# albireo77/moonrtx

Hardware: AMD Instinct MI355X
Metric: Mrays/s (primary camera samples) at 3840x2160, 64 spp, downscale-2 DEM (higher is better)
Workload: dtype f32

## Files before the change

moonrtx_amd/csrc/mrtx_kernels.hip:

```cpp
#include <hip/hip_runtime.h>
#include <stdint.h>
#include <string.h>
#include <stdlib.h>
#include <type_traits>

#include "mrtx_device.h"
#include "mrtx_march.h"

namespace mrtx {

#ifdef MRTX_PROF
__device__ unsigned long long g_prof[16];
#endif

__device__ __forceinline__ uint32_t mix32(uint32_t x) {
    x ^= x >> 16; x *= 0x7feb352dU;
    x ^= x >> 15; x *= 0x846ca68bU;
    x ^= x >> 16;
    return x;
}
__device__ __forceinline__ float u01(uint32_t key, uint32_t dim) {
    const uint32_t r = mix32(key + (dim + 1u) * 0x9E3779B9u);
    return (float)(r >> 8) * 5.9604644775390625e-08f;
}
// ... 165 lines not shown
        if (!have) {
            const bool far_end = !(y <= 0.0f);
            const float q0 = far_end ? o0 - ba0 : o0, q1 = far_end ? o1 - ba1 : o1, q2 = far_end ? o2 - ba2 : o2;
            const float B2 = fmaf(dz, q2, fmaf(dy, q1, dx * q0));
            const float C2 = fmaf(q2, q2, fmaf(q1, q1, q0 * q0)) - rr;
            const float h2 = fmaf(B2, B2, -C2);
            if (h2 > 0.0f) { cand = -B2 - sqrtf(h2); have = true; }
        }
        if (have) {
            const float sc = ta + cand;
            if (sc > smin && sc < best) { best = sc; which = k; }
        }
    }
    return which >= 0 ? best : -1.0e30f;
}


__device__ __forceinline__ void env_rowcol(const FrameC& f, float fx, float fy, float& rowf, float& colf) {
    const float sx = fmaf(fx, CF(f)->two_over_w, -1.0f);
    const float sy = fmaf(-fy, CF(f)->two_over_h, 1.0f);
    float dx = fmaf(sy, CF(f)->Vy[0], fmaf(sx, CF(f)->Ux[0], CF(f)->Wd[0]));
    float dy = fmaf(sy, CF(f)->Vy[1], fmaf(sx, CF(f)->Ux[1], CF(f)->Wd[1]));
    float dz = fmaf(sy, CF(f)->Vy[2], fmaf(sx, CF(f)->Ux[2], CF(f)->Wd[2]));
    const float inv_len = rcp_cr(sqrt_sh(fmaf(dz, dz, fmaf(dy, dy, dx * dx))));
    dx = dx * inv_len; dy = dy * inv_len; dz = dz * inv_len;
    float el, az;
    latlon(dx, dy, dz, fmaf(dy, dy, dx * dx), el, az);
    rowf = fmaf(el, CF(f)->bg_row_scale, CF(f)->bg_row_off);
    colf = fmaf(az, CF(f)->bg_col_scale, CF(f)->bg_col_off);
}
__device__ __forceinline__ bool sky_pixel_uniform(const FrameC& f, int x, int y, float& e0, float& e1, float& e2) {
    float r00, c00, r10, c10, r01, c01, r11, c11;
    const float fx = (float)x, fy = (float)y;
    env_rowcol(f, fx, fy, r00, c00);
    env_rowcol(f, fx + 1.0f, fy, r10, c10);
    env_rowcol(f, fx, fy + 1.0f, r01, c01);
    env_rowcol(f, fx + 1.0f, fy + 1.0f, r11, c11);
    const float m = fmaf(1.0e-6f, (float)max(CF(f)->bg_w, CF(f)->bg_h), 0.02f);
    const float rlo = fminf(fminf(r00, r10), fminf(r01, r11)) - m, rhi = fmaxf(fmaxf(r00, r10), fmaxf(r01, r11)) + m;
    const float clo = fminf(fminf(c00, c10), fminf(c01, c11)) - m, chi = fmaxf(fmaxf(c00, c10), fmaxf(c01, c11)) + m;
    const float rf = floorf(rlo), cf = floorf(clo);
    const bool uni = rf == floorf(rhi) && cf == floorf(chi) && rlo >= 0.0f && clo >= 0.0f &&
                     rhi < (float)CF(f)->bg_h && chi < (float)CF(f)->bg_w;
    e0 = e1 = e2 = 0.0f;
    if (uni) {
        const uint32_t px = reinterpret_cast<const uint32_t*>(CF(f)->bg)[(int64_t)(int)rf * CF(f)->bg_w + (int)cf];
        e0 = (float)(px & 255u) * kInv255;
        e1 = (float)((px >> 8) & 255u) * kInv255;
        e2 = (float)((px >> 16) & 255u) * kInv255;
    }
    return uni;
}

#define MRTX_PARK_SLOTS 4
__device__ __forceinline__ void park_put(v4f* park, int slot, float a, float b, float c, float d) {
    const v4f v = {a, b, c, d};
    park[slot * 64 + threadIdx.x] = v;
}
__device__ __forceinline__ v4f park_get(const v4f* park, int slot) { return park[slot * 64 + threadIdx.x]; }
__device__ __forceinline__ void park_fence() { asm volatile("" ::: "memory"); }

struct SampleOut {
    float c0, c1, c2, hitflag;
    float h0, h1, h2, h3;
    float oa, ob, oc, da, db, dc, t0, t1, t2, row, col;
    uint32_t ks, aux;
    bool path;
};

template <bool STATS, bool WIDE, int MODE, bool OVERLAY>
__device__ __forceinline__ void trace_sample(const FrameC& f, int lt, int x, int y, uint32_t gs, SampleOut& o,
                                             uint32_t* cnt, bool lead = false, v4f* park = nullptr) {
    constexpr bool BOUNCE = MODE == 1, DEFER = MODE == 2;
    auto emit_hit = [&](float h0, float h1, float h2, float h3) {
        if (DEFER) {
            if (lead) reinterpret_cast<float4*>(CF(f)->hits)[(int64_t)y * f.W + x] = make_float4(h0, h1, h2, h3);
        } else {
            o.h0 = h0; o.h1 = h1; o.h2 = h2; o.h3 = h3;
        }
    };
    constexpr int BATCH = BOUNCE ? MRTX_STEP_BATCH_BOUNCE : MRTX_STEP_BATCH;
    const uint32_t pix = (uint32_t)y * (uint32_t)f.W + (uint32_t)x;
    const uint32_t kp = mix32(pix + CF(f)->key0);
    const uint32_t ks = mix32(kp ^ (gs * 0x85EBCA6Bu + 1u));
    const float u0 = u01(ks, 0), u1 = u01(ks, 1), u2 = u01(ks, 2), u3 = u01(ks, 3);
    o.c0 = o.c1 = o.c2 = 0.0f; o.hitflag = 0.0f;
    o.h0 = o.h1 = o.h2 = o.h3 = 0.0f;
    o.path = false;
    if (DEFER) { o.oa = o.ob = o.oc = o.da = o.db = o.dc = o.t0 = o.t1 = o.t2 = o.row = o.col = 0.0f; o.ks = 0u; o.aux = 0u; }
    if (STATS) cnt[ST_PRIMARY]++;
    PROF_BEGIN(1);

    const float fx = (float)x + u0, fy = (float)y + u1;
    const float sx = fmaf(fx, CF(f)->two_over_w, -1.0f);
    const float sy = fmaf(-fy, CF(f)->two_over_h, 1.0f);
    float dx = fmaf(sy, CF(f)->Vy[0], fmaf(sx, CF(f)->Ux[0], CF(f)->Wd[0]));
    float dy = fmaf(sy, CF(f)->Vy[1], fmaf(sx, CF(f)->Ux[1], CF(f)->Wd[1]));
    float dz = fmaf(sy, CF(f)->Vy[2], fmaf(sx, CF(f)->Ux[2], CF(f)->Wd[2]));
    const float inv_len = rcp_cr(sqrt_sh(fmaf(dz, dz, fmaf(dy, dy, dx * dx))));
    dx = dx * inv_len; dy = dy * inv_len; dz = dz * inv_len;
    if (MODE == 3) {
        if (CF(f)->bg) env_lookup<STATS>(f, dx, dy, dz, o.c0, o.c1, o.c2, cnt);
        emit_hit(0.0f, 0.0f, 0.0f, 0.0f);
        return;
    }

    const double Dx = (double)dx, Dy = (double)dy, Dz = (double)dz;
    const double a = (Dx * Dx + Dy * Dy) + Dz * Dz;
    const double b = (CF(f)->oc[0] * Dx + CF(f)->oc[1] * Dy) + CF(f)->oc[2] * Dz;
    const double disc = b * b - a * CF(f)->cq;
    bool on_sphere = false;
    double t0 = 0.0, t1 = 0.0;
    if (disc > 0.0) {
        const double sq = (double)sqrtf((float)disc);
        const double inva = (double)rcp_cr((float)a);
        t0 = (-b - sq) * inva;
        t1 = (-b + sq) * inva;
        if (t1 > 0.0) { on_sphere = true; if (t0 < 0.0) t0 = 0.0; }
    }
    int cap = -1;
    float cap_s = 0.0f, cr0 = 0.0f, cr1 = 0.0f, cr2 = 0.0f;
    double tc0 = 0.0;
    bool cap_front = false;
    if (OVERLAY) {
        tc0 = -b * (double)rcp_cr((float)a);
// ... 64 lines not shown
             CF(f)->centerf[1] + fmaf(v.pc, CF(f)->Mf[2][1], fmaf(v.pb, CF(f)->Mf[1][1], v.pa * CF(f)->Mf[0][1])),
             CF(f)->centerf[2] + fmaf(v.pc, CF(f)->Mf[2][2], fmaf(v.pb, CF(f)->Mf[1][2], v.pa * CF(f)->Mf[0][2])),
             (float)t0 + lo);

    float t0r = 1.0f, t1r = 1.0f, t2r = 1.0f;
    uint32_t seg = 1;
    float ul1 = u2, ul2 = u3;
    uint32_t ksl = ks;
    float org_row = 0.0f, org_col = 0.0f, org_cell = 0.0f;
    for (;;) {
        PROF_BEGIN(5);
        float wgt;
        if (DEFER) {
            float oa, ob, oc, wa, wb, wc, carried = 0.0f;
            const bool have_s = light_sample(f, v, ul1, ul2, oa, ob, oc, wa, wb, wc, carried);
            float q2o;
            exact_rowcol(f, oa, ob, oc, org_row, org_col, q2o);
            org_cell = CF(f)->hmip != nullptr ? horizon_cell(f, org_row, org_col) : 0.0f;
            park_put(park, 3, org_row, org_col, org_cell, 0.0f);
            park_put(park, 0, v.pa, v.pb, v.pc, v.na);
            park_put(park, 1, v.nb, v.nc, v.al0, v.al1);
            park_put(park, 2, v.al2, __uint_as_float(ksl), carried, 0.0f);
            park_fence();
            bool occluded = false;
            if (have_s) {
                if (STATS) cnt[ST_SHADOW]++;
                Seg ssg;
                float sk_occ;
                MarchState ms;
                ms.rowA = org_row; ms.colA = org_col;
                bool sgo = march_begin_at<false, STATS, false, true>(f, oa, ob, oc, wa, wb, wc, ms, cnt, org_cell);
                while (sgo) march_segment<WIDE, false, STATS, MRTX_SHADOW_BATCH, 2>(f, ms, 0.0f, ssg, sgo, occluded, sk_occ, cnt);
            }
            park_fence();
            { const v4f p3 = park_get(park, 3); org_row = p3.x; org_col = p3.y; org_cell = p3.z; }
            const v4f p0 = park_get(park, 0), p1 = park_get(park, 1), p2 = park_get(park, 2);
            v.pa = p0.x; v.pb = p0.y; v.pc = p0.z; v.na = p0.w;
            v.nb = p1.x; v.nc = p1.y; v.al0 = p1.z; v.al1 = p1.w;
            v.al2 = p2.x; ksl = __float_as_uint(p2.y);
            wgt = (have_s && !occluded) ? p2.z : 0.0f;
        } else {
            wgt = direct_light<STATS, WIDE, BATCH>(f, v, ul1, ul2, cnt);
        }
        PROF_END(5);
        o.c0 = fmaf(t0r * v.al0, wgt, o.c0);
        o.c1 = fmaf(t1r * v.al1, wgt, o.c1);
        o.c2 = fmaf(t2r * v.al2, wgt, o.c2);
        if (DEFER) {
            if (continue_path(f, v, ksl, 1u, t0r, t1r, t2r, o.oa, o.ob, o.oc, o.da, o.db, o.dc)) {
                o.row = org_row; o.col = org_col;
                o.t0 = t0r; o.t1 = t1r; o.t2 = t2r;
                o.ks = ksl; o.aux = 0u;
                if (STATS) cnt[ST_BOUNCE]++;
#ifdef MRTX_PROF
                uint32_t tcnt[16];
#pragma unroll
                for (int i = 0; i < 16; i++) tcnt[i] = 0;
#else
                uint32_t tcnt_store[STATS ? ST_N : 1];
                uint32_t* const tcnt = STATS ? tcnt_store : nullptr;
#endif
                if (STATS) {
#pragma unroll
                    for (int i = 0; i < ST_N; i++) tcnt[i] = 0;
                }
                MarchState tm;
                tm.rowA = o.row; tm.colA = o.col;
                park_put(park, 0, o.c0, o.c1, o.c2, o.t0);
                park_put(park, 1, o.t1, o.t2, __uint_as_float(o.ks), 0.0f);
                park_fence();
                bool tgo = march_begin_at<false, STATS, false, true>(f, o.oa, o.ob, o.oc, o.da, o.db, o.dc, tm, tcnt, org_cell);
                bool thit = false;
                Seg tsg;
                float tsk = 0.0f;
                if (tgo) march_segment<WIDE, false, STATS, MRTX_TRIAL_BATCH, 3>(f, tm, 0.0f, tsg, tgo, thit, tsk, tcnt);
                park_fence();
                const v4f p0 = park_get(park, 0), p1 = park_get(park, 1);
                o.c0 = p0.x; o.c1 = p0.y; o.c2 = p0.z; o.t0 = p0.w;
                o.t1 = p1.x; o.t2 = p1.y; o.ks = __float_as_uint(p1.z);
                t0r = o.t0; t1r = o.t1; t2r = o.t2;
#ifdef MRTX_PROF_TRIAL
                cnt[13] += tcnt[11]; cnt[14] += tcnt[12]; cnt[15] += tcnt[6] + tcnt[7];
#endif
                if (STATS) {
#pragma unroll
                    for (int i = 0; i < ST_N; i++) cnt[i] += tcnt[i];
                }
                if (!tgo && !thit) {
                    escaped_path<STATS>(f, o.oa, o.ob, o.oc, o.da, o.db, o.dc, t0r, t1r, t2r, o.c0, o.c1, o.c2, cnt);
                } else {
                    o.path = true;
                    if (thit) {
                        o.aux = MRTX_REC_HIT | ((uint32_t)(int)rintf(tsk * f.inv_step) << 8);
                    } else {
                        o.aux = MRTX_REC_RESUME | ((uint32_t)tm.kend << 8);
                        o.row = tm.rowA; o.col = tm.colA;
                    }
                }
            }
        }
        if (!BOUNCE) break;
        float boa, bob, boc, bda, bdb, bdc;
        if (!continue_path(f, v, ks, seg, t0r, t1r, t2r, boa, bob, boc, bda, bdb, bdc)) break;
        const uint32_t d0 = 4u + 5u * (seg - 1u);
        ul1 = u01(ks, d0 + 3u); ul2 = u01(ks, d0 + 4u);
        if (STATS) cnt[ST_BOUNCE]++;
        Seg bsg;
        float bhi = 0.0f;
        if (!march<WIDE, false, STATS, BATCH>(f, boa, bob, boc, bda, bdb, bdc, 0.0f, bsg, bhi, cnt)) {
            escaped_path<STATS>(f, boa, bob, boc, bda, bdb, bdc, t0r, t1r, t2r, o.c0, o.c1, o.c2, cnt);
            break;
        }
        const int bk = (int)rintf(bhi * f.inv_step);
        float blo = (float)(bk - 1) * f.step;
        refine<WIDE>(f, bsg, boa, bob, boc, bda, bdb, bdc, blo, bhi);
        if (STATS) { cnt[ST_HEIGHT] += (uint32_t)f.nbis; cnt[ST_FETCH] += (uint32_t)f.nbis; }
        hit_vertex<STATS, WIDE>(f, fmaf(blo, bda, boa), fmaf(blo, bdb, bob), fmaf(blo, bdc, boc), v, cnt);
        seg++;
    }
}

template <int S>
__device__ __forceinline__ float tree_sum(float v) {
#pragma unroll
    for (int m = 1; m < S; m <<= 1) v += __shfl_xor(v, m, 64);
    return v;
}

#ifndef MRTX_WG_TILE
#define MRTX_WG_TILE 1
#endif
#ifndef MRTX_SKY_WG_TILE
#define MRTX_SKY_WG_TILE 8
#endif
#ifndef MRTX_MIN_WAVES
#define MRTX_MIN_WAVES 4
#endif
#ifndef MRTX_XCD_SHARE
#define MRTX_XCD_SHARE 1
#endif
#ifndef MRTX_XCD_TILE_RUN
#define MRTX_XCD_TILE_RUN 1
#endif
#ifndef MRTX_XCD_SHARE_BELOW
#define MRTX_XCD_SHARE_BELOW 1200
#endif
#ifndef MRTX_MIN_WAVES_BOUNCE
#define MRTX_MIN_WAVES_BOUNCE 5
#endif
#ifndef MRTX_BOUNCE_STATS_WAVES
#define MRTX_BOUNCE_STATS_WAVES 2
#endif
#define MRTX_BOUNCE_WAVES(STATS, SV) ((STATS) ? MRTX_BOUNCE_STATS_WAVES : ((SV) <= 2 ? 4 : MRTX_MIN_WAVES_BOUNCE))
template <int S, bool STATS, bool WIDE, int MODE, bool OVERLAY>
#ifndef MRTX_MIN_WAVES_DEFER
#define MRTX_MIN_WAVES_DEFER 3
#endif
__global__ void __launch_bounds__(64, MODE == 1 ? MRTX_BOUNCE_WAVES(STATS, S) : MODE == 2 ? MRTX_MIN_WAVES_DEFER : MRTX_MIN_WAVES)
render_kernel(const FrameC f, const PathQ pq) {
    constexpr bool DEFER = MODE == 2;
    constexpr int P = 64 / S;
    constexpr int PW = P >= 64 ? 8 : P >= 32 ? 8 : P >= 16 ? 4 : P >= 8 ? 4 : P >= 4 ? 2 : P >= 2 ? 2 : 1;
    constexpr int PH = P / PW;
    constexpr int WGTILE = MODE == 3 ? MRTX_SKY_WG_TILE : MRTX_WG_TILE;
    constexpr int WGT = (PW > WGTILE) ? PW : WGTILE;
    constexpr int WGS = WGT == 16 ? 4 : WGT == 8 ? 3 : WGT == 4 ? 2 : WGT == 2 ? 1 : 0;
    constexpr int JX = WGT / PW, JY = WGT / PH, NJOBS = JX * JY;
    __shared__ unsigned int lds_cnt[ST_N];
    __shared__ v4f park_lds[DEFER ? MRTX_PARK_SLOTS * 64 : 1];
    v4f* const park = DEFER ? park_lds : nullptr;

    const int lane = threadIdx.x & 63, wv = threadIdx.x >> 6;
    const int subs_x = f.tile_w >> WGS, subs = subs_x * (f.tile_h >> WGS);
    const int b = blockIdx.x, xcd = b & 7, g = b >> 3;
    int li, sub;
    if (f.xcd_share) {
        const int per = subs >> 3;
        li = g / per; sub = xcd * per + g % per;
    } else {
        constexpr int K = MRTX_XCD_TILE_RUN;
        const int rem = g % (subs * K);
        li = ((g / (subs * K)) * 8 + xcd) * K + rem / subs; sub = rem % subs;
    }
    if (li >= f.n_active) return;
    const int lt = f.tile_list ? f.tile_list[li] : li;
    const int t = lt * f.world + f.rank;
    int tx, ty;
    mrtx_tile_xy(t, f.tiles_x, f.tile_shift, tx, ty);
    const int px0 = tx * f.tile_w + (sub % subs_x) * WGT, py0 = ty * f.tile_h + (sub / subs_x) * WGT;
    if (px0 >= f.W || py0 >= f.H) return;

#ifdef MRTX_PROF
    uint32_t cnt[16];
    if (!STATS) {
#pragma unroll
        for (int i = 0; i < 16; i++) cnt[i] = 0;
    }
#else
    uint32_t cnt_store[STATS ? ST_N : 1];
    uint32_t* const cnt = STATS ? cnt_store : nullptr;
#endif
    if (STATS) {
#pragma unroll
        for (int i = 0; i < ST_N; i++) cnt[i] = 0;
        if (threadIdx.x < ST_N) lds_cnt[threadIdx.x] = 0;
        __syncthreads();
    }

    const int p = lane / S, s = lane % S;
    constexpr bool SKY_UNI = MODE == 3 && WGT == 8;
    uint64_t sky_nu = ~0ull;
    auto sky_jobmask = [&](int jx_, int jy_) {
        uint64_t mk = 0ull;
#pragma unroll
        for (int r = 0; r < PH; r++) mk |= (uint64_t)((1u << PW) - 1u) << ((jy_ * PH + r) * 8 + jx_ * PW);
        return mk;
    };
    if (SKY_UNI && CF(f)->bg != nullptr) {
        const int ux = px0 + (lane & 7), uy = py0 + (lane >> 3);
        const bool uin = ux < f.W && uy < f.H;
        float sky0, sky1, sky2;
        const bool uni = sky_pixel_uniform(f, ux, uy, sky0, sky1, sky2);
        sky_nu = __ballot(uin && !uni);
        if (uin && (sky_nu & sky_jobmask((lane & 7) / PW, (lane >> 3) / PH)) == 0ull) {
            const int64_t upix = (int64_t)uy * f.W + ux;
            float4 a = make_float4(0.f, 0.f, 0.f, 0.f);
            if (f.first_block != 0) a = reinterpret_cast<const float4*>(CF(f)->accum)[upix];
            const float b0 = (float)S * sky0, b1 = (float)S * sky1, b2 = (float)S * sky2;
            a.x += b0; a.y += b1; a.z += b2; a.w += 0.0f;
            reinterpret_cast<float4*>(CF(f)->accum)[upix] = a;
            reinterpret_cast<float4*>(CF(f)->hits)[upix] = make_float4(0.f, 0.f, 0.f, 0.f);
            if (STATS) { cnt[ST_PRIMARY] += (uint32_t)S; cnt[ST_BG] += (uint32_t)S; }
        }
    }
    for (int job = wv; job < NJOBS; job++) {
        const int jx = job % JX, jy = job / JX;
        const int x = px0 + jx * PW + (p % PW), y = py0 + jy * PH + (p / PW);
        if (px0 + jx * PW >= f.W || py0 + jy * PH >= f.H) continue;
        if (SKY_UNI && (sky_nu & sky_jobmask(jx, jy)) == 0ull) continue;
        const bool inb = x < f.W && y < f.H;
        float s0 = 0.f, s1 = 0.f, s2 = 0.f, s3 = 0.f;
        SampleOut o;
        o.h0 = o.h1 = o.h2 = o.h3 = 0.f;
        o.path = false;
        o.oa = o.ob = o.oc = o.da = o.db = o.dc = o.t0 = o.t1 = o.t2 = o.row = o.col = 0.f; o.ks = 0u; o.aux = 0u;
        bool deferred = false;
        constexpr uint32_t n_blk = 1u;
        for (uint32_t blk = 0; blk < n_blk; blk++) {
            o.c0 = o.c1 = o.c2 = o.hitflag = 0.f;
            PROF_BEGIN(0);
            if (inb) trace_sample<STATS, WIDE, MODE, OVERLAY>(f, lt, x, y, (f.first_block + blk) * (uint32_t)S + (uint32_t)s, o, cnt, s == 0, park);
            PROF_END(0);
            if (blk == 0 && f.first_block != 0 && inb && s == 0) {
                const float4 prev = reinterpret_cast<const float4*>(CF(f)->accum)[(int64_t)y * f.W + x];
                s0 = prev.x; s1 = prev.y; s2 = prev.z; s3 = prev.w;
            }
            if (DEFER) deferred = __ballot(o.path) != 0ull;
            if (DEFER && deferred) {
                const uint32_t chunk = (uint32_t)blockIdx.x * (uint32_t)NJOBS + (uint32_t)job;
                const uint32_t e = chunk * 64u + (uint32_t)lane;
                const uint64_t pm = __ballot(o.path);
                const uint32_t es = chunk * 64u + __builtin_amdgcn_mbcnt_hi((uint32_t)(pm >> 32), __builtin_amdgcn_mbcnt_lo((uint32_t)pm, 0u));
                if (o.path) {
                    nt_store4(pq.ray0 + es, o.oa, o.ob, o.oc, o.da);
                    nt_store4(pq.ray1 + es, o.db, o.dc, o.t0, o.t1);
                    nt_store4(pq.ray2 + es, o.t2, o.row, o.col, __uint_as_float(o.ks));
                    pq.lane_of[es] = (uint32_t)lane | o.aux;
                }
                { float* const cp = reinterpret_cast<float*>(pq.c4) + 3u * (size_t)e;
                  __builtin_nontemporal_store(o.c0, cp); __builtin_nontemporal_store(o.c1, cp + 1); __builtin_nontemporal_store(o.c2, cp + 2); }
                if (lane == 0) pq.npaths[chunk] = (uint8_t)__popcll(pm);
                if (lane == 0) pq.meta[chunk] = 0x80000000u | (uint32_t)(px0 + jx * PW) | ((uint32_t)(py0 + jy * PH) << 15);
            } else {
                s0 += tree_sum<S>(o.c0);
                s1 += tree_sum<S>(o.c1);
                s2 += tree_sum<S>(o.c2);
            }
            s3 += tree_sum<S>(o.hitflag);
        }
        if (inb && s == 0) reinterpret_cast<float4*>(CF(f)->accum)[(int64_t)y * f.W + x] = make_float4(s0, s1, s2, s3);
        if (!DEFER && inb && s == 0) reinterpret_cast<float4*>(CF(f)->hits)[(int64_t)y * f.W + x] = make_float4(o.h0, o.h1, o.h2, o.h3);
    }

#ifdef MRTX_PROF
    if (!STATS && lane == 0 && (((uint32_t)(blockIdx.x >> 3) * 2654435761u) >> 26) == 0u) {
        cnt[10] = 1;
#pragma unroll
        for (int i = 0; i < 16; i++) atomicAdd(&g_prof[i], (unsigned long long)cnt[i]);
    }
#endif
    if (STATS) {
#pragma unroll
        for (int i = 0; i < ST_N; i++) {
            uint32_t v = cnt[i];
#pragma unroll
            for (int m = 1; m < 64; m <<= 1) v += __shfl_xor(v, m, 64);
            if (lane == 0) atomicAdd(&lds_cnt[i], v);
        }
        __syncthreads();
        if (threadIdx.x < ST_N) atomicAdd(&CF(f)->stats[threadIdx.x], (unsigned long long)lds_cnt[threadIdx.x]);
    }
}

#ifndef MRTX_PATH_WAVES
#define MRTX_PATH_WAVES 5
#endif
#ifndef MRTX_PATH_STEPS
#define MRTX_PATH_STEPS 2
#endif
#ifdef MRTX_PATH_PROF
__device__ unsigned long long g_pprof[16];
__device__ unsigned long long g_pprof_end[8192];
__device__ unsigned long long g_pprof_t[16];
#endif
enum { PS_IDLE = 0, PS_NEEDSEG, PS_STEP, PS_BISECT, PS_ENDED, PS_HITWAIT, PS_SHADE, PS_ESCAPED };

template <bool STATS>
__device__ __forceinline__ uint32_t step_mask(const FrameC& f, const MarchState& m, const Seg& sg, uint32_t todo, uint32_t* cnt) {
    const float* m2 = CF(f)->mip2;
    const int pitch = CF(f)->m2_pitch, sh = CF(f)->m2_shift, mh = CF(f)->m2_h, mw = CF(f)->m2_w;
    uint32_t rem = todo, keep = 0u;
    while (rem != 0u) {
        int jj[4]; bool on[4]; float mv[4];
#pragma unroll
        for (int q = 0; q < 4; q++) {
            on[q] = rem != 0u;
            jj[q] = on[q] ? (int)__builtin_ctz(rem) + 1 : 1;
            rem &= rem - 1u;
        }
#pragma unroll
        for (int q = 0; q < 4; q++) {
            const float u = ((float)(m.ka + jj[q]) * f.step - sg.sa) * f.inv_step;
            const float rowf = fmaf(u, fmaf(u, sg.r2, sg.r1), sg.ra), colf = fmaf(u, fmaf(u, sg.c2, sg.c1), sg.ca);
            int i = ((int)floorf(rowf) >> sh) + 1, c = ((int)floorf(colf) >> sh) + 1;
            i = max(0, min(i, mh + 1)); c = max(0, min(c, mw + 1));
            mv[q] = on[q] ? m2[i * pitch + c] : 0.0f;
        }
        if (STATS) { cnt[ST_MIP] += (on[0] ? 1u : 0u) + (on[1] ? 1u : 0u) + (on[2] ? 1u : 0u) + (on[3] ? 1u : 0u); }
#pragma unroll
        for (int q = 0; q < 4; q++) {
            const float sk = (float)(m.ka + jj[q]) * f.step;
            const float pa = fmaf(sk, m.da, m.oa), pb = fmaf(sk, m.db, m.ob), pc = fmaf(sk, m.dc, m.oc);
            const float r2 = fmaf(pc, pc, fmaf(pb, pb, pa * pa));
            const float rd = f.Rf * mv[q];
            if (on[q] && r2 <= (rd * rd) * 1.00001f) keep |= 1u << (jj[q] - 1);
        }
    }
    return keep;
}

template <bool STATS, bool WIDE>
__global__ void __launch_bounds__(64, STATS ? 2 : MRTX_PATH_WAVES) path_kernel(const FrameC f, const PathQ pq) {
    const uint32_t lane = threadIdx.x;
    const uint32_t label = blockIdx.x & 7u;
    const uint32_t sub = (blockIdx.x >> 3) % (uint32_t)pq.n_sub;
// ... 725 lines not shown
        int i = t / mp - 1, j = t % mp - 1;
        i = i < 0 ? 0 : (i > mh - 1 ? mh - 1 : i);
        j = j < 0 ? mw - 1 : (j > mw - 1 ? 0 : j);
        const int r0 = max(C * i - 2, -2), r1 = min(C * i + C + 1, h + 1);
        const int c0 = max(C * j - 2, -2), c1 = min(C * j + C + 1, w + 1);
        float m = 0.0f;
        for (int r = r0; r <= r1; r++) {
            const float* row = dem_padded + ((int64_t)(r + 2) * pitch + 2) * (MRTX_DEM_ELEM_BYTES / 4);
            for (int c = c0; c <= c1; c++) m = fmaxf(m, row[c * (MRTX_DEM_ELEM_BYTES / 4)]);
        }
        mip[t] = m;
    }
}

__global__ void hmip_build_kernel(const float* __restrict__ mip, int mh, int mw, int shift, float* __restrict__ out,
                                  int hh, int hw, int hshift, int h, int w) {
    const int mp = mw + 2, Cc = 1 << hshift;
    for (int t = blockIdx.x * blockDim.x + threadIdx.x; t < hh * hw; t += gridDim.x * blockDim.x) {
        const int i = t / hw, j = t % hw;
        const int r0 = max(Cc * i - Cc, 0), r1 = min(Cc * i + 2 * Cc - 1, h - 1);
        const int c0 = Cc * j - Cc, c1 = Cc * j + 2 * Cc - 1;
        float m = 0.0f;
        int a0 = 0, a1 = mw - 1, b0 = 1, b1 = 0;
        if (c1 - c0 + 1 < w) {
            if (c0 < 0)       { a0 = (c0 + w) >> shift; a1 = mw - 1; b0 = 0; b1 = c1 >> shift; }
            else if (c1 >= w) { a0 = c0 >> shift; a1 = mw - 1; b0 = 0; b1 = (c1 - w) >> shift; }
            else              { a0 = c0 >> shift; a1 = c1 >> shift; }
        }
        for (int fi = r0 >> shift; fi <= (r1 >> shift); fi++) {
            for (int fj = a0; fj <= a1; fj++) m = fmaxf(m, mip[(fi + 1) * mp + fj + 1]);
            for (int fj = b0; fj <= b1; fj++) m = fmaxf(m, mip[(fi + 1) * mp + fj + 1]);
        }
        out[t] = m;
    }
}

__global__ void mip_pair_kernel(const float* __restrict__ mip, float2* __restrict__ out, int rows, int pitch) {
    const int n = rows * pitch;
    for (int t = blockIdx.x * blockDim.x + threadIdx.x; t < n; t += gridDim.x * blockDim.x) {
        const int r = t / pitch;
        out[t] = make_float2(mip[t], mip[r + 1 < rows ? t + pitch : t]);
    }
}

}

#ifdef MRTX_DEV_ONE
#ifndef MRTX_DEV_ONE_MODE
#define MRTX_DEV_ONE_MODE 2
#endif
#if MRTX_DEV_ONE_MODE == 9
template __global__ void mrtx::path_kernel<false, true>(const FrameC, const PathQ);
#else
template __global__ void mrtx::render_kernel<64, false, true, MRTX_DEV_ONE_MODE, false>(const FrameC, const PathQ);
#endif
#else
extern "C++" {
static void render_geometry(const FrameC& f, int S, int& xcd_share, unsigned& grid, int& njobs, int& pw_log2, int mode = 0) {
    const int P = 64 / S;
    const int PW = P >= 32 ? 8 : P >= 8 ? 4 : P >= 2 ? 2 : 1;
    const int PH = P / PW;
    const int wgtile = mode == 3 ? MRTX_SKY_WG_TILE : MRTX_WG_TILE;
    const int wgt = (PW > wgtile) ? PW : wgtile;
    const int subs = (f.tile_w / wgt) * (f.tile_h / wgt);
    xcd_share = (MRTX_XCD_SHARE && (subs & 7) == 0 && f.n_active < MRTX_XCD_SHARE_BELOW) ? 1 : 0;
    const int groups = xcd_share ? f.n_active : (f.n_active + 8 * MRTX_XCD_TILE_RUN - 1) / (8 * MRTX_XCD_TILE_RUN) * (8 * MRTX_XCD_TILE_RUN);
    grid = (unsigned)(groups * subs);
    njobs = (wgt / PW) * (wgt / PH);
    pw_log2 = PW == 8 ? 3 : PW == 4 ? 2 : PW == 2 ? 1 : 0;
}
uint64_t mrtx_path_chunks(const FrameC& f, int S, uint32_t* grid_a, int* njobs_log2) {
    int share, njobs, pwl; unsigned grid;
    render_geometry(f, S, share, grid, njobs, pwl);
    if (grid_a) *grid_a = grid;
    if (njobs_log2) *njobs_log2 = njobs == 2 ? 1 : 0;
    return (uint64_t)grid * (uint64_t)njobs;
}
hipError_t mrtx_launch_render(const FrameC& f, int S, bool stats, int mode, bool overlay, const PathQ* pq, hipStream_t st) {
    FrameC fr = f;
    int njobs, pwl; unsigned gx;
    render_geometry(f, S, fr.xcd_share, gx, njobs, pwl, mode);
    const dim3 grid(gx), block(64);
    if (f.n_blocks != 1) return hipErrorInvalidValue;
    if (grid.x == 0) return hipSuccess;
    PathQ q;
    memset(&q, 0, sizeof q);
    if (mode == 2) {
        if (!pq || pq->n_chunks != (uint64_t)gx * (uint64_t)njobs || pq->grid_a != gx || (1 << pq->njobs_log2) != njobs)
            return hipErrorInvalidValue;
        q = *pq;
    }
    const bool wide = f.dem_wide != 0;
    static const unsigned dev_lds = getenv("MOONRT_DEV_LDS") ? (unsigned)atoi(getenv("MOONRT_DEV_LDS")) : 0u;
#define MRTX_LAUNCH(SV, ST, WD, MD, OV) hipLaunchKernelGGL((mrtx::render_kernel<SV, ST, WD, MD, OV>), grid, block, dev_lds, st, fr, q)
#define MRTX_CASE3(SV, MD, OV)                                                                                     \
        if (wide) { if (stats) MRTX_LAUNCH(SV, true, true, MD, OV); else MRTX_LAUNCH(SV, false, true, MD, OV); }   \
        else { if (stats) MRTX_LAUNCH(SV, true, false, MD, OV); else MRTX_LAUNCH(SV, false, false, MD, OV); }
#define MRTX_CASE2(SV, MD) if (overlay) { MRTX_CASE3(SV, MD, true) } else { MRTX_CASE3(SV, MD, false) }
#define MRTX_CASE(SV)                                                  \
    case SV:                                                           \
        if (mode == 1) { MRTX_CASE2(SV, 1) } else if (mode == 2) { MRTX_CASE2(SV, 2) }                              \
        else if (mode == 3) { if (stats) MRTX_LAUNCH(SV, true, false, 3, false); else MRTX_LAUNCH(SV, false, false, 3, false); }   \
        else { MRTX_CASE2(SV, 0) }   \
        break;
    switch (S) {
#ifndef MRTX_DEV_ONLY_S64
        MRTX_CASE(1) MRTX_CASE(2) MRTX_CASE(4) MRTX_CASE(8) MRTX_CASE(16) MRTX_CASE(32)
// ... 206 lines not shown
```

moonrtx_amd/csrc/mrtx_march.h:

```cpp
#pragma once
#include <hip/hip_runtime.h>
#include <stdint.h>

#include "mrtx_device.h"

#define CF(f) ((const __attribute__((address_space(4))) FrameCold*)(f).cold)

#ifndef MRTX_TRIAL_BATCH
#define MRTX_TRIAL_BATCH 1
#endif

namespace mrtx {

__device__ constexpr float kPi = 3.14159274101257324f;
__device__ constexpr float kHalfPi = 1.57079637050628662f;
__device__ constexpr float kInv255 = 0.003921568859368563f;

#ifdef MRTX_PROF
#ifdef MRTX_PROF_FULLIV
#define PROF_BEGIN(i)
#define PROF_END(i)
#else
#define PROF_BEGIN(i) const unsigned long long _pt##i = __builtin_readcyclecounter()
#define PROF_END(i) cnt[i] += (uint32_t)(__builtin_readcyclecounter() - _pt##i)
// ... 469 lines not shown
            mv[q] = m2[min((uint32_t)((i + 1) * pitch + c + 1), maxidx)];
        }
        bool found = false;
#pragma unroll
        for (int q = 0; q < Q; q++) {
            const int jj = j - q;
            const float sk = fmaf((float)max(jj, sg.jlo), f.step, sg.sa);
            const float r2 = fmaf(sk, fmaf(sk, m.rq.a, two_b), m.rq.q0);
            const float rd = f.Rf * mv[q];
            const bool kept = !(r2 > (rd * rd) * 1.00001f);
            if (STATS) cnt[ST_MIP] += (!found && jj >= sg.jlo) ? 1u : 0u;
            if (!found && jj >= sg.jlo && kept) { last = jj; found = true; }
        }
        j -= Q;
        open = !found && j >= sg.jlo;
    }
    return last;
}
template <bool STATS, int Q>
__device__ __forceinline__ int first_kept_step(const FrameC& f, const MarchState& m, const Seg& sg, uint32_t* cnt) {
    const float* m2 = CF(f)->mip2;
    const int pitch = CF(f)->m2_pitch, sh = CF(f)->m2_shift;
    const uint32_t maxidx = (uint32_t)((CF(f)->m2_h + 2) * pitch - 1);
    const float two_b = m.rq.b + m.rq.b;
    int j = sg.jlo;
    int first = sg.jlo;
    bool open = (sg.jlo <= sg.jhi) & !sg.exact;
    if (open) first = sg.jhi + 1;
    while (open) {
        float mv[Q];
#pragma unroll
        for (int q = 0; q < Q; q++) {
            const float u = (float)min(j + q, sg.jhi);
            const float rowf = fmaf(u, fmaf(u, sg.r2, sg.r1), sg.ra), colf = fmaf(u, fmaf(u, sg.c2, sg.c1), sg.ca);
            const int i = (int)floorf(rowf) >> sh, c = (int)floorf(colf) >> sh;
            mv[q] = m2[min((uint32_t)((i + 1) * pitch + c + 1), maxidx)];
        }
        bool found = false;
#pragma unroll
        for (int q = 0; q < Q; q++) {
            const int jj = j + q;
            const float sk = fmaf((float)min(jj, sg.jhi), f.step, sg.sa);
            const float r2 = fmaf(sk, fmaf(sk, m.rq.a, two_b), m.rq.q0);
            const float rd = f.Rf * mv[q];
            const bool kept = !(r2 > (rd * rd) * 1.00001f);
            if (STATS) cnt[ST_MIP] += (!found && jj <= sg.jhi) ? 1u : 0u;
            if (!found && jj <= sg.jhi && kept) { first = jj; found = true; }
        }
        j += Q;
        open = !found && j <= sg.jhi;
    }
    return first;
}
template <bool WIDE, bool PRIMARY, bool STATS, int BATCH, int SCAN = PRIMARY ? 1 : 0, bool BOUNDED = false>
__device__ __forceinline__ void march_segment(const FrameC& f, MarchState& m, float smax, Seg& sg, bool& go, bool& hit,
                                              float& sk_hit, uint32_t* cnt) {
    const float oa = m.oa, ob = m.ob, oc = m.oc, da = m.da, db = m.db, dc = m.dc;
    const int ka = m.ka;
    float rowB, colB, q2B;
    if (!PRIMARY && (MRTX_HORIZON_RETRY & 1) != 0 && ka > 0 && m.kend >= f.kmax) {
        const int ke = horizon_retry(f, m);
        if (ke < 1) {
            if (STATS) cnt[ST_HEIGHT] += steps_after<BOUNDED>(f, m, ka + 1, smax);
            go = false;
            return;
        }
        m.kend = min(f.kmax, ka + ke);
    }
    PROF_BEGIN(6);
    seg_setup<STATS>(f, oa, ob, oc, da, db, dc, m.rq, ka, m.rowA, m.colA, m.q2A, sg, rowB, colB, q2B, cnt);
#ifdef MRTX_PROF_FULLIV
    { const bool full = (sg.jlo == 1) & (sg.jhi == SEG_N) & !sg.exact;
      cnt[13] += (uint32_t)__popcll(__ballot(full)); cnt[14] += (uint32_t)__popcll(__ballot(sg.exact));
      cnt[5] += (uint32_t)__popcll(__ballot(full && sg.why == 1)); cnt[6] += (uint32_t)__popcll(__ballot(full && sg.why == 2));
      cnt[7] += (uint32_t)__popcll(__ballot(full && sg.why == 3)); }
#endif
    if (!PRIMARY) sg.jhi = max(min(sg.jhi, m.kend - ka), sg.jlo - 1);
    if (SCAN == 1 && (MRTX_SEG_MASK & 4) != 0 && CF(f)->mip2 != nullptr) sg.jlo = first_kept_step<STATS, MRTX_PMASK_Q>(f, m, sg, cnt);
    if (SCAN == 2 && (MRTX_SEG_MASK & 2) != 0 && CF(f)->mip2 != nullptr) sg.jhi = last_kept_step<STATS, MRTX_PMASK_Q>(f, m, sg, cnt);
    if (SCAN == 3 && (MRTX_SEG_MASK & 1) != 0 && CF(f)->mip2 != nullptr) sg.jhi = last_kept_step<STATS, MRTX_PMASK_Q>(f, m, sg, cnt);
    PROF_END(6);
    PROF_BEGIN(7);
    if (STATS) cnt[ST_HEIGHT] += count_in_steps<PRIMARY, BOUNDED>(f, oa, ob, oc, da, db, dc, smax, ka, 1, sg.jlo - 1);
    if (__ballot(sg.exact) != 0ull)
        step_loop<WIDE, PRIMARY, STATS, true, 1, BOUNDED>(f, oa, ob, oc, da, db, dc, smax, sg, ka, go, hit, sk_hit, cnt);
    else
        step_loop<WIDE, PRIMARY, STATS, false, BATCH, BOUNDED>(f, oa, ob, oc, da, db, dc, smax, sg, ka, go, hit, sk_hit, cnt);
    PROF_END(7);
#ifdef MRTX_PROF
#if !defined(MRTX_PROF_TRIAL) && !defined(MRTX_PROF_FULLIV)
    cnt[8] += 1;
    cnt[9] += (uint32_t)__popcll(__ballot(true));
    cnt[PRIMARY ? 13 : 14] += (__ballot(sg.jlo <= sg.jhi) == 0ull) ? 1u : 0u;
    cnt[15] += PRIMARY ? 1u : 0u;
#endif
#ifdef MRTX_PROF_FULLIV
    cnt[8] += 1; cnt[9] += (uint32_t)__popcll(__ballot(true));
#endif
#endif
    segment_tail<PRIMARY, STATS, BOUNDED>(f, m, smax, sg, go, rowB, colB, q2B, cnt);
}

template <bool WIDE, bool PRIMARY, bool STATS, int BATCH, int SCAN = PRIMARY ? 1 : 0, bool BOUNDED = false>
__device__ __forceinline__ bool march(const FrameC& f, float oa, float ob, float oc, float da, float db, float dc,
                                      float smax, Seg& sg, float& sk_hit, uint32_t* cnt) {
    MarchState m;
    bool hit = false;
    bool go = march_begin<PRIMARY, STATS, false, BOUNDED>(f, oa, ob, oc, da, db, dc, m, cnt, smax);
    while (go) march_segment<WIDE, PRIMARY, STATS, BATCH, SCAN, BOUNDED>(f, m, smax, sg, go, hit, sk_hit, cnt);
    return hit;
}

template <bool WIDE>
__device__ __forceinline__ void refine(const FrameC& f, const Seg& sg, float oa, float ob, float oc, float da, float db,
                                       float dc, float& lo, float& hi) {
    auto below = [&](float s) {
        const float ma = fmaf(s, da, oa), mb = fmaf(s, db, ob), mc = fmaf(s, dc, oc);
        return below_seg<WIDE, true>(f, sg, s, ma, mb, mc, fmaf(mc, mc, fmaf(mb, mb, ma * ma)));
    };
    for (int i = 0; i < f.nbis; i++) {
        const float mid = 0.5f * (lo + hi);
        const bool bel = below(mid);
        hi = bel ? mid : hi;
        lo = bel ? lo : mid;
    }
}

struct Vertex {
    float pa, pb, pc;
    float na, nb, nc;
    float al0, al1, al2;
};

__device__ __forceinline__ void duff_basis(float na, float nb, float nc, float& b1a, float& b1b, float& b1c, float& b2a,
                                           float& b2b, float& b2c) {
    const float sg = nc >= 0.0f ? 1.0f : -1.0f;
    const float aa = -rcp_cr(sg + nc);
    const float bb = (na * nb) * aa;
    b1a = fmaf(sg, (na * na) * aa, 1.0f); b1b = sg * bb; b1c = -sg * na;
    b2a = bb; b2b = fmaf(nb * nb, aa, sg); b2c = -nb;
}

template <bool STATS, bool WIDE>
__device__ __forceinline__ void hit_vertex(const FrameC& f, float ha, float hb, float hc, Vertex& v, uint32_t* cnt) {
    const float rho2 = fmaf(hb, hb, ha * ha);
    const float r2 = fmaf(hc, hc, rho2);
    const float rho = sqrt_sh(rho2);
    const float r = sqrt_sh(r2);
    float lat, lon;
    latlon(ha, hb, hc, rho2, lat, lon);
    const float rowf = fmaf(lat, f.gd.row_scale, f.gd.row_off);
    const float colf = fmaf(lon, f.gd.col_scale, f.gd.col_off);
    const float dn = dem_march<WIDE>(f, rowf - 1.0f, colf);
// ... 91 lines not shown
```

Measured before the change: 30330.

## Spread deferred trial-march steps across wave lanes via LDS work redistribution

Moves the trial shadow/bounce march in defer mode out of the per-sample trace into the render loop. Each lane first runs a few private steps, then the remaining step counts are compacted across the wave: ray parameters go into the LDS park area and all 64 lanes evaluate consecutive steps of different rays in parallel, with ballots picking the first terminating step. The goal is to cut idle lanes caused by uneven step counts in divergent loops. It adds LDS traffic, an extra park slot, wave barriers, and a tighter SGPR limit on the defer kernel, which may raise spilling or register pressure.

```diff
diff --git a/moonrtx_amd/csrc/mrtx_kernels.hip b/moonrtx_amd/csrc/mrtx_kernels.hip
--- a/moonrtx_amd/csrc/mrtx_kernels.hip
+++ b/moonrtx_amd/csrc/mrtx_kernels.hip
@@ -241,7 +241,7 @@
     return uni;
 }
 
-#define MRTX_PARK_SLOTS 4
+#define MRTX_PARK_SLOTS (MRTX_TRIAL_WIDE ? 5 : 4)
 __device__ __forceinline__ void park_put(v4f* park, int slot, float a, float b, float c, float d) {
     const v4f v = {a, b, c, d};
     park[slot * 64 + threadIdx.x] = v;
@@ -257,9 +257,38 @@
     bool path;
 };
 
+struct TrialState {
+    MarchState m;
+    Seg sg;
+    float rowB, colB, q2B;
+    float sk;
+    int stage;
+#ifdef MRTX_PROF
+    uint32_t tc[16];
+#endif
+};
+template <bool STATS>
+__device__ __forceinline__ void trial_finish(const FrameC& f, SampleOut& o, MarchState& tm, bool tgo, bool thit, float tsk,
+                                             const v4f* park, uint32_t* cnt) {
+    const v4f p0 = park_get(park, 0), p1 = park_get(park, 1);
+    o.c0 = p0.x; o.c1 = p0.y; o.c2 = p0.z; o.t0 = p0.w;
+    o.t1 = p1.x; o.t2 = p1.y; o.ks = __float_as_uint(p1.z);
+    if (!tgo && !thit) {
+        escaped_path<STATS>(f, o.oa, o.ob, o.oc, o.da, o.db, o.dc, o.t0, o.t1, o.t2, o.c0, o.c1, o.c2, cnt);
+    } else {
+        o.path = true;
+        if (thit) {
+            o.aux = MRTX_REC_HIT | ((uint32_t)(int)rintf(tsk * f.inv_step) << 8);
+        } else {
+            o.aux = MRTX_REC_RESUME | ((uint32_t)tm.kend << 8);
+            o.row = tm.rowA; o.col = tm.colA;
+        }
+    }
+}
+
 template <bool STATS, bool WIDE, int MODE, bool OVERLAY>
 __device__ __forceinline__ void trace_sample(const FrameC& f, int lt, int x, int y, uint32_t gs, SampleOut& o,
-                                             uint32_t* cnt, bool lead = false, v4f* park = nullptr) {
+                                             uint32_t* cnt, bool lead = false, v4f* park = nullptr, TrialState* tw = nullptr) {
     constexpr bool BOUNCE = MODE == 1, DEFER = MODE == 2;
     auto emit_hit = [&](float h0, float h1, float h2, float h3) {
         if (DEFER) {
@@ -430,6 +459,25 @@
                 o.t0 = t0r; o.t1 = t1r; o.t2 = t2r;
                 o.ks = ksl; o.aux = 0u;
                 if (STATS) cnt[ST_BOUNCE]++;
+#if MRTX_TRIAL_WIDE
+                park_put(park, 0, o.c0, o.c1, o.c2, o.t0);
+                park_put(park, 1, o.t1, o.t2, __uint_as_float(o.ks), 0.0f);
+                park_fence();
+                TrialState& t = *tw;
+#ifdef MRTX_PROF
+                uint32_t* const tcnt = t.tc;
+#else
+                uint32_t* const tcnt = cnt;
+#endif
+                t.m.rowA = o.row; t.m.colA = o.col;
+                bool tgo = march_begin_at<false, STATS, false, true>(f, o.oa, o.ob, o.oc, o.da, o.db, o.dc, t.m, tcnt, org_cell);
+                t.stage = 1;
+                if (tgo) {
+                    segment_head<false, STATS, 3, false>(f, t.m, 0.0f, t.sg, tgo, t.rowB, t.colB, t.q2B, tcnt);
+                    t.stage = t.sg.exact ? 3 : 2;
+                    if (STATS) tcnt[ST_HEIGHT] += count_in_steps<false>(f, o.oa, o.ob, o.oc, o.da, o.db, o.dc, 0.0f, 0, 1, t.sg.jlo - 1);
+                }
+#else
 #ifdef MRTX_PROF
                 uint32_t tcnt[16];
 #pragma unroll
@@ -453,28 +501,27 @@
                 float tsk = 0.0f;
                 if (tgo) march_segment<WIDE, false, STATS, MRTX_TRIAL_BATCH, 3>(f, tm, 0.0f, tsg, tgo, thit, tsk, tcnt);
                 park_fence();
-                const v4f p0 = park_get(park, 0), p1 = park_get(park, 1);
-                o.c0 = p0.x; o.c1 = p0.y; o.c2 = p0.z; o.t0 = p0.w;
-                o.t1 = p1.x; o.t2 = p1.y; o.ks = __float_as_uint(p1.z);
-                t0r = o.t0; t1r = o.t1; t2r = o.t2;
 #ifdef MRTX_PROF_TRIAL
-                cnt[13] += tcnt[11]; cnt[14] += tcnt[12]; cnt[15] += tcnt[6] + tcnt[7];
+                {
+                    const uint32_t mine = tcnt[11];
+                    uint32_t iters = 0u, steps = 0u;
+                    bool top = true;
+#pragma unroll
+                    for (int b = 4; b >= 0; b--) {
+                        const bool bit = ((mine >> b) & 1u) != 0u;
+                        steps += (uint32_t)__popcll(__ballot(bit)) << b;
+                        if (__ballot(top && bit) != 0ull) { iters |= 1u << b; top = top && bit; }
+                    }
+                    if ((int)(threadIdx.x & 63u) == __ffsll((long long)__ballot(true)) - 1) { cnt[13] += iters; cnt[14] += steps; }
+                    cnt[15] += tcnt[6] + tcnt[7];
+                }
 #endif
                 if (STATS) {
 #pragma unroll
                     for (int i = 0; i < ST_N; i++) cnt[i] += tcnt[i];
                 }
-                if (!tgo && !thit) {
-                    escaped_path<STATS>(f, o.oa, o.ob, o.oc, o.da, o.db, o.dc, t0r, t1r, t2r, o.c0, o.c1, o.c2, cnt);
-                } else {
-                    o.path = true;
-                    if (thit) {
-                        o.aux = MRTX_REC_HIT | ((uint32_t)(int)rintf(tsk * f.inv_step) << 8);
-                    } else {
-                        o.aux = MRTX_REC_RESUME | ((uint32_t)tm.kend << 8);
-                        o.row = tm.rowA; o.col = tm.colA;
-                    }
-                }
+                trial_finish<STATS>(f, o, tm, tgo, thit, tsk, park, cnt);
+#endif
             }
         }
         if (!BOUNCE) break;
@@ -530,12 +577,13 @@
 #define MRTX_BOUNCE_STATS_WAVES 2
 #endif
 #define MRTX_BOUNCE_WAVES(STATS, SV) ((STATS) ? MRTX_BOUNCE_STATS_WAVES : ((SV) <= 2 ? 4 : MRTX_MIN_WAVES_BOUNCE))
-template <int S, bool STATS, bool WIDE, int MODE, bool OVERLAY>
 #ifndef MRTX_MIN_WAVES_DEFER
 #define MRTX_MIN_WAVES_DEFER 3
 #endif
-__global__ void __launch_bounds__(64, MODE == 1 ? MRTX_BOUNCE_WAVES(STATS, S) : MODE == 2 ? MRTX_MIN_WAVES_DEFER : MRTX_MIN_WAVES)
-render_kernel(const FrameC f, const PathQ pq) {
+#define MRTX_RENDER_BOUNDS(S, STATS, MODE) \
+    __launch_bounds__(64, (MODE) == 1 ? MRTX_BOUNCE_WAVES(STATS, S) : (MODE) == 2 ? MRTX_MIN_WAVES_DEFER : MRTX_MIN_WAVES)
+template <int S, bool STATS, bool WIDE, int MODE, bool OVERLAY>
+__device__ __forceinline__ void render_body(const FrameC& f, const PathQ& pq) {
     constexpr bool DEFER = MODE == 2;
     constexpr int P = 64 / S;
     constexpr int PW = P >= 64 ? 8 : P >= 32 ? 8 : P >= 16 ? 4 : P >= 8 ? 4 : P >= 4 ? 2 : P >= 2 ? 2 : 1;
@@ -627,7 +675,63 @@
         for (uint32_t blk = 0; blk < n_blk; blk++) {
             o.c0 = o.c1 = o.c2 = o.hitflag = 0.f;
             PROF_BEGIN(0);
+#if MRTX_TRIAL_WIDE
+            TrialState ts;
+            ts.stage = 0;
+            ts.sk = 0.0f;
+            ts.sg.jlo = 1; ts.sg.jhi = 0;
+#ifdef MRTX_PROF
+#pragma unroll
+            for (int i = 0; i < 16; i++) ts.tc[i] = 0;
+            uint32_t* const tcnt = ts.tc;
+#else
+            uint32_t* const tcnt = cnt;
+#endif
+            if (inb) trace_sample<STATS, WIDE, MODE, OVERLAY>(f, lt, x, y, (f.first_block + blk) * (uint32_t)S + (uint32_t)s, o, cnt, s == 0, park, &ts);
+            if (DEFER) {
+                const bool live = ts.stage >= 2;
+                bool tgo = live, thit = false;
+                ts.sg.exact = ts.stage == 3;
+                if (__ballot(live) != 0ull) {
+#ifdef MRTX_PROF
+                    const unsigned long long pt7 = __builtin_readcyclecounter();
+#endif
+                    trial_steps_wide<WIDE, STATS>(f, ts.m, ts.sg, live, park + 2 * 64, reinterpret_cast<uint32_t*>(park + 64) + 3,
+                                                  tgo, thit, ts.sk, tcnt);
+#ifdef MRTX_PROF
+                    tcnt[7] += (uint32_t)(__builtin_readcyclecounter() - pt7);
+#endif
+                }
+                if (ts.stage != 0) {
+                    if (live) segment_tail<false, STATS>(f, ts.m, 0.0f, ts.sg, tgo, ts.rowB, ts.colB, ts.q2B, tcnt);
+                    park_fence();
+#ifdef MRTX_PROF
+                    if (STATS) {
+#pragma unroll
+                        for (int i = 0; i < ST_N; i++) cnt[i] += tcnt[i];
+                    }
+#endif
+                    trial_finish<STATS>(f, o, ts.m, tgo, thit, ts.sk, park, cnt);
+                }
+#ifdef MRTX_PROF_TRIAL
+                {
+                    const uint32_t mine = tcnt[11];
+                    uint32_t iters = 0u, steps = 0u;
+                    bool top = true;
+#pragma unroll
+                    for (int b = 4; b >= 0; b--) {
+                        const bool bit = ((mine >> b) & 1u) != 0u;
+                        steps += (uint32_t)__popcll(__ballot(bit)) << b;
+                        if (__ballot(top && bit) != 0ull) { iters |= 1u << b; top = top && bit; }
+                    }
+                    if (lane == 0) { cnt[13] += iters; cnt[14] += steps; }
+                    cnt[8] += tcnt[8]; cnt[9] += tcnt[9]; cnt[15] += tcnt[6] + tcnt[7];
+                }
+#endif
+            }
+#else
             if (inb) trace_sample<STATS, WIDE, MODE, OVERLAY>(f, lt, x, y, (f.first_block + blk) * (uint32_t)S + (uint32_t)s, o, cnt, s == 0, park);
+#endif
             PROF_END(0);
             if (blk == 0 && f.first_block != 0 && inb && s == 0) {
                 const float4 prev = reinterpret_cast<const float4*>(CF(f)->accum)[(int64_t)y * f.W + x];
@@ -661,6 +765,15 @@
     }
 
 #ifdef MRTX_PROF
+#ifdef MRTX_PROF_TRIAL
+    if (!STATS) {
+#pragma unroll
+        for (int i = 13; i <= 14; i++) {
+#pragma unroll
+            for (int m = 1; m < 64; m <<= 1) cnt[i] += __shfl_xor(cnt[i], m, 64);
+        }
+    }
+#endif
     if (!STATS && lane == 0 && (((uint32_t)(blockIdx.x >> 3) * 2654435761u) >> 26) == 0u) {
         cnt[10] = 1;
 #pragma unroll
@@ -679,6 +792,21 @@
         if (threadIdx.x < ST_N) atomicAdd(&CF(f)->stats[threadIdx.x], (unsigned long long)lds_cnt[threadIdx.x]);
     }
 }
+template <int S, bool STATS, bool WIDE, int MODE, bool OVERLAY>
+__global__ void MRTX_RENDER_BOUNDS(S, STATS, MODE) render_kernel(const FrameC f, const PathQ pq) {
+    render_body<S, STATS, WIDE, MODE, OVERLAY>(f, pq);
+}
+#if MRTX_TRIAL_WIDE
+#ifndef MRTX_DEFER_SGPRS
+#define MRTX_DEFER_SGPRS 96
+#endif
+#define MRTX_DEFER_TIGHT(WD, OV)                                                                                                 \
+    template <> __global__ void __attribute__((amdgpu_num_sgpr(MRTX_DEFER_SGPRS))) MRTX_RENDER_BOUNDS(64, false, 2)              \
+    render_kernel<64, false, WD, 2, OV>(const FrameC f, const PathQ pq) { render_body<64, false, WD, 2, OV>(f, pq); }
+MRTX_DEFER_TIGHT(false, false)
+MRTX_DEFER_TIGHT(true, false)
+#undef MRTX_DEFER_TIGHT
+#endif
 
 #ifndef MRTX_PATH_WAVES
 #define MRTX_PATH_WAVES 5
@@ -1510,7 +1638,9 @@
 #if MRTX_DEV_ONE_MODE == 9
 template __global__ void mrtx::path_kernel<false, true>(const FrameC, const PathQ);
 #else
+#if !(MRTX_TRIAL_WIDE && MRTX_DEV_ONE_MODE == 2)
 template __global__ void mrtx::render_kernel<64, false, true, MRTX_DEV_ONE_MODE, false>(const FrameC, const PathQ);
+#endif
 #endif
 #else
 extern "C++" {
diff --git a/moonrtx_amd/csrc/mrtx_march.h b/moonrtx_amd/csrc/mrtx_march.h
--- a/moonrtx_amd/csrc/mrtx_march.h
+++ b/moonrtx_amd/csrc/mrtx_march.h
@@ -545,18 +545,17 @@
     }
     return first;
 }
-template <bool WIDE, bool PRIMARY, bool STATS, int BATCH, int SCAN = PRIMARY ? 1 : 0, bool BOUNDED = false>
-__device__ __forceinline__ void march_segment(const FrameC& f, MarchState& m, float smax, Seg& sg, bool& go, bool& hit,
-                                              float& sk_hit, uint32_t* cnt) {
+template <bool PRIMARY, bool STATS, int SCAN, bool BOUNDED>
+__device__ __forceinline__ bool segment_head(const FrameC& f, MarchState& m, float smax, Seg& sg, bool& go, float& rowB, float& colB,
+                                             float& q2B, uint32_t* cnt) {
     const float oa = m.oa, ob = m.ob, oc = m.oc, da = m.da, db = m.db, dc = m.dc;
     const int ka = m.ka;
-    float rowB, colB, q2B;
     if (!PRIMARY && (MRTX_HORIZON_RETRY & 1) != 0 && ka > 0 && m.kend >= f.kmax) {
         const int ke = horizon_retry(f, m);
         if (ke < 1) {
             if (STATS) cnt[ST_HEIGHT] += steps_after<BOUNDED>(f, m, ka + 1, smax);
             go = false;
-            return;
+            return false;
         }
         m.kend = min(f.kmax, ka + ke);
     }
@@ -573,6 +572,15 @@
     if (SCAN == 2 && (MRTX_SEG_MASK & 2) != 0 && CF(f)->mip2 != nullptr) sg.jhi = last_kept_step<STATS, MRTX_PMASK_Q>(f, m, sg, cnt);
     if (SCAN == 3 && (MRTX_SEG_MASK & 1) != 0 && CF(f)->mip2 != nullptr) sg.jhi = last_kept_step<STATS, MRTX_PMASK_Q>(f, m, sg, cnt);
     PROF_END(6);
+    return true;
+}
+template <bool WIDE, bool PRIMARY, bool STATS, int BATCH, int SCAN = PRIMARY ? 1 : 0, bool BOUNDED = false>
+__device__ __forceinline__ void march_segment(const FrameC& f, MarchState& m, float smax, Seg& sg, bool& go, bool& hit,
+                                              float& sk_hit, uint32_t* cnt) {
+    const float oa = m.oa, ob = m.ob, oc = m.oc, da = m.da, db = m.db, dc = m.dc;
+    const int ka = m.ka;
+    float rowB, colB, q2B;
+    if (!segment_head<PRIMARY, STATS, SCAN, BOUNDED>(f, m, smax, sg, go, rowB, colB, q2B, cnt)) return;
     PROF_BEGIN(7);
     if (STATS) cnt[ST_HEIGHT] += count_in_steps<PRIMARY, BOUNDED>(f, oa, ob, oc, da, db, dc, smax, ka, 1, sg.jlo - 1);
     if (__ballot(sg.exact) != 0ull)
@@ -592,6 +600,129 @@
 #endif
 #endif
     segment_tail<PRIMARY, STATS, BOUNDED>(f, m, smax, sg, go, rowB, colB, q2B, cnt);
+}
+
+#ifndef MRTX_TRIAL_WIDE
+#define MRTX_TRIAL_WIDE 1
+#endif
+#ifndef MRTX_TRIAL_WIDE_K
+#define MRTX_TRIAL_WIDE_K 5
+#endif
+#ifndef MRTX_TRIAL_WIDE_MIN
+#define MRTX_TRIAL_WIDE_MIN 2
+#endif
+typedef float xch4 __attribute__((ext_vector_type(4)));
+__device__ __forceinline__ void xch_order() {
+    __builtin_amdgcn_fence(__ATOMIC_RELEASE, "workgroup");
+    __builtin_amdgcn_wave_barrier();
+    __builtin_amdgcn_fence(__ATOMIC_ACQUIRE, "workgroup");
+}
+template <bool WIDE>
+__device__ __forceinline__ void trial_step(const FrameC& f, float ra, float r1, float r2, float ca, float c1, float c2, float oa,
+                                           float ob, float oc, float da, float db, float dc, int k, bool& in, bool& bel) {
+    const float sk = (float)k * f.step;
+    const float pa = fmaf(sk, da, oa), pb = fmaf(sk, db, ob), pc = fmaf(sk, dc, oc);
+    const float q = fmaf(pc, pc, fmaf(pb, pb, pa * pa));
+    in = (q <= f.R2f) & (k <= f.kmax);
+    const float u = (sk - 0.0f) * f.inv_step;
+    const float rowf = fmaf(u, fmaf(u, r2, r1), ra);
+    const float colf = fmaf(u, fmaf(u, c2, c1), ca);
+    const float surf = f.Rf * dem_march<WIDE>(f, rowf, colf);
+    bel = q <= surf * surf;
+}
+template <bool WIDE, bool STATS>
+__device__ __forceinline__ void trial_steps_wide(const FrameC& f, const MarchState& m, const Seg& sg, bool live, xch4* st,
+                                                 uint32_t* ctl, bool& go, bool& hit, float& sk_out, uint32_t* cnt) {
+    if (__ballot(live && sg.exact) != 0ull) {
+        if (live) step_loop<WIDE, false, STATS, true, 1>(f, m.oa, m.ob, m.oc, m.da, m.db, m.dc, 0.0f, sg, 0, go, hit, sk_out, cnt);
+        return;
+    }
+    const uint32_t lane = threadIdx.x & 63u;
+    const int jhi = live ? sg.jhi : 0;
+    int j = live ? sg.jlo : 1;
+    bool pend = j <= jhi;
+#pragma unroll
+    for (int it = 0; it < MRTX_TRIAL_WIDE_K; it++) {
+        if (pend) {
+            bool in, bel;
+            trial_step<WIDE>(f, sg.ra, sg.r1, sg.r2, sg.ca, sg.c1, sg.c2, m.oa, m.ob, m.oc, m.da, m.db, m.dc, j, in, bel);
+            if (STATS) { cnt[ST_HEIGHT] += in ? 1u : 0u; cnt[ST_FETCH]++; }
+#ifdef MRTX_PROF
+            cnt[11] += 1;
+#endif
+            hit = in & bel; go = in & !bel; sk_out = (float)j * f.step;
+            j++;
+            pend = go & (j <= jhi);
+        }
+    }
+    uint32_t n, start, W, nmax;
+    auto deal = [&]() {
+        n = pend ? (uint32_t)(jhi - j + 1) : 0u;
+        start = 0u; W = 0u; nmax = 0u;
+        bool top = true;
+#pragma unroll
+        for (int b = 4; b >= 0; b--) {
+            const bool bit = ((n >> b) & 1u) != 0u;
+            const uint64_t mk = __ballot(bit);
+            start += __builtin_amdgcn_mbcnt_hi((uint32_t)(mk >> 32), __builtin_amdgcn_mbcnt_lo((uint32_t)mk, 0u)) << b;
+            W += (uint32_t)__popcll(mk) << b;
+            if (__ballot(top && bit) != 0ull) { nmax |= 1u << b; top = top && bit; }
+        }
+    };
+    deal();
+    if (W == 0u) return;
+    if (((int)nmax - MRTX_TRIAL_WIDE_MIN) * 64 <= (int)W) {
+        step_loop_from<WIDE, false, STATS, false, 1>(f, m.oa, m.ob, m.oc, m.da, m.db, m.dc, 0.0f, sg, 0, j, pend, go, hit, sk_out, cnt);
+        return;
+    }
+    const uint64_t rays = __ballot(n > 0u);
+    const uint32_t c = __builtin_amdgcn_mbcnt_hi((uint32_t)(rays >> 32), __builtin_amdgcn_mbcnt_lo((uint32_t)rays, 0u));
+    uint16_t* const c16 = reinterpret_cast<uint16_t*>(ctl);
+    if (lane < 32u) ctl[lane * 4u] = 0u;
+    xch_order();
+    if (n > 0u) {
+        const xch4 a = {sg.ra, sg.r1, sg.r2, sg.ca}, b = {sg.c1, sg.c2, m.oa, m.ob}, cc = {m.oc, m.da, m.db, m.dc};
+        st[c] = a; st[64u + c] = b; st[128u + c] = cc;
+        c16[(32u + (c >> 1)) * 8u + (c & 1u)] = (uint16_t)(start | ((uint32_t)j << 10));
+        __hip_atomic_fetch_or(&ctl[(start >> 5) * 4u], 1u << (start & 31u), __ATOMIC_RELAXED, __HIP_MEMORY_SCOPE_WORKGROUP);
+    }
+    xch_order();
+    const uint64_t lanes_le = (2ull << lane) - 1ull;
+    uint32_t before = 0u;
+    for (uint32_t base = 0u;; base += 64u) {
+        const uint32_t h0 = (uint32_t)__builtin_amdgcn_readfirstlane((int)ctl[(base >> 5) * 4u]);
+        const uint32_t h1 = (uint32_t)__builtin_amdgcn_readfirstlane((int)ctl[((base >> 5) + 1u) * 4u]);
+        const uint64_t heads = ((uint64_t)h1 << 32) | h0;
+        const uint32_t ci = (before + (uint32_t)__popcll(heads & lanes_le) - 1u) & 63u;
+        const uint32_t t = base + lane;
+        const uint32_t sj = c16[(32u + (ci >> 1)) * 8u + (ci & 1u)];
+        const int jj = min((int)((sj >> 10) + (t - (sj & 1023u))), SEG_N);
+#ifdef MRTX_PROF_TRIAL
+        if (lane == 0u) { cnt[8] += 1u; cnt[9] += min(W - base, 64u); }
+#endif
+        const xch4 a = st[ci], b = st[64u + ci], cc = st[128u + ci];
+        bool in, bel;
+        trial_step<WIDE>(f, a.x, a.y, a.z, a.w, b.x, b.y, b.z, b.w, cc.x, cc.y, cc.z, cc.w, jj, in, bel);
+        const uint64_t term = __ballot((t < W) & !(in & !bel)), inside = __ballot(in);
+        if (pend && start < base + 64u) {
+            const uint32_t p0 = start > base ? start - base : 0u, p1 = min(start + n - base, 64u);
+            const uint64_t mine = term & ~((1ull << p0) - 1ull) & (p1 >= 64u ? ~0ull : (1ull << p1) - 1ull);
+            if (mine != 0ull) {
+                const uint32_t p = (uint32_t)__ffsll((long long)mine) - 1u;
+                const int jt = j + (int)(base + p - start);
+                hit = ((inside >> p) & 1ull) != 0ull;
+                go = false;
+                sk_out = (float)jt * f.step;
+                if (STATS) { cnt[ST_FETCH] += (uint32_t)(jt - j + 1); cnt[ST_HEIGHT] += (uint32_t)(jt - j) + (hit ? 1u : 0u); }
+                pend = false;
+            } else if (start + n <= base + 64u) {
+                if (STATS) { cnt[ST_FETCH] += n; cnt[ST_HEIGHT] += n; }
+                pend = false;
+            }
+        }
+        if (__ballot(pend) == 0ull) break;
+        before += (uint32_t)__popc(h0) + (uint32_t)__popc(h1);
+    }
 }
 
 template <bool WIDE, bool PRIMARY, bool STATS, int BATCH, int SCAN = PRIMARY ? 1 : 0, bool BOUNDED = false>
```

Measured after the change: 30720, median of 6. +1.3%, better.
